# mgp25/OpenLTE

Hardware: AMD Instinct MI355X
Metric: DL subframes/sec @20MHz 100RB 64QAM, full chain FFT->CE->demap->rate-unmatch->turbo(REF)->CRC (SURVEY 8d W4) (higher is better)
Workload: dtype i8 IQ in, f32 FFT/CE/equaliser, i8 soft bits, i16 path metrics (differences exact modulo 2^16); 1 GPU; W4 full DL chain: 20 MHz/100 RB/64QAM, 9 allocations per subframe (8x12 PRB TBS 3240 + 1x4 PRB TBS 1064), 65536 subframes per GPU, int8 IQ in HBM; subframes_per_gpu=65536, N_ant=1, CFI=2, channel_estimate_form=compact, decoder=REF (reference-faithful, bit-exact), unique_subframes=96, streams_per_gpu=1

## Files before the change

### openlte_amd/csrc/turbo.hip

```cpp
#include <algorithm>
#include <cstring>
#include <initializer_list>
#include <type_traits>
#include <vector>

#include "plan_core.hpp"

using namespace turbo_geom;

namespace {

constexpr uint32_t RX_NULL_AS_INT = 10000;


__device__ __forceinline__ int sbyte(uint32_t w, int k) { return (int)__builtin_amdgcn_sbfe(w, 8 * k, 8); }

typedef __attribute__((address_space(3))) const uint8_t  lds_u8_t;
typedef __attribute__((address_space(3))) const int8_t   lds_i8_t;
typedef __attribute__((address_space(3))) const uint16_t lds_u16_t;
__device__ __forceinline__ uint32_t lds_u8(uint32_t addr) { return *(lds_u8_t *)(uintptr_t)addr; }
__device__ __forceinline__ int      lds_i8(uint32_t addr) { return *(lds_i8_t *)(uintptr_t)addr; }
__device__ __forceinline__ uint32_t lds_u16(uint32_t addr) { return *(lds_u16_t *)(uintptr_t)addr; }

typedef short v2s __attribute__((ext_vector_type(2)));
__device__ __forceinline__ v2s      as_v2s(uint32_t w) { return __builtin_bit_cast(v2s, w); }
__device__ __forceinline__ uint32_t as_u32(v2s v) { return __builtin_bit_cast(uint32_t, v); }
__device__ __forceinline__ v2s      even2(uint32_t w) { return (as_v2s(w) << 8) >> 8; }
__device__ __forceinline__ v2s      odd2(uint32_t w) { return as_v2s(w) >> 8; }
__device__ __forceinline__ uint32_t merge_bytes(v2s e, v2s o) { return __builtin_amdgcn_perm(as_u32(o), as_u32(e), 0x06020400u); }
__device__ __forceinline__ v2s      abs2(v2s a) { return __builtin_elementwise_max(a, (v2s)(0) - a); }
__device__ __forceinline__ uint32_t neg_mask(v2s d)
{
    uint32_t m;
    asm("v_pk_ashrrev_i16 %0, 15, %1 op_sel_hi:[0,1]" : "=v"(m) : "v"(as_u32(d)));
    return m;
}
__device__ __forceinline__ v2s bit_select(uint32_t m, v2s yes, v2s no) { return as_v2s((as_u32(yes) & m) | (as_u32(no) & ~m)); }
__device__ __forceinline__ v2s half_sum(v2s a, v2s b)
{
    uint32_t t = as_u32(a + b);
    asm("" : "+v"(t));
    return as_v2s(t) >> 1;
}

__device__ __forceinline__ int soft_xor(int a, int b)
{
    int mag = (abs(a) + abs(b)) >> 1;
    return ((a < 0) != (b < 0)) ? -mag : mag;
}


template <typename Op> __device__ __forceinline__ int wave_reduce_i(int v, Op op)
{
    v = op(v, __builtin_amdgcn_update_dpp(v, v, 0xB1, 0xF, 0xF, false));
    v = op(v, __builtin_amdgcn_update_dpp(v, v, 0x4E, 0xF, 0xF, false));
    v = op(v, __builtin_amdgcn_update_dpp(v, v, 0x141, 0xF, 0xF, false));
    v = op(v, __builtin_amdgcn_update_dpp(v, v, 0x140, 0xF, 0xF, false));
    return op(op(__builtin_amdgcn_readlane(v, 0), __builtin_amdgcn_readlane(v, 16)), op(__builtin_amdgcn_readlane(v, 32), __builtin_amdgcn_readlane(v, 48)));
}
__device__ __forceinline__ int      wave_max_i(int v) { return wave_reduce_i(v, [](int a, int b) { return max(a, b); }); }
__device__ __forceinline__ uint32_t wave_xor_u(uint32_t v) { return (uint32_t)wave_reduce_i((int)v, [](int a, int b) { return a ^ b; }); }
__device__ __forceinline__ float    wave_max_f(float v)
{
    return __int_as_float(wave_max_i(__float_as_int(v)));
}

__device__ __forceinline__ float block_max_abs_f(float v, float *red )
{
    v = wave_max_f(v);
    __syncthreads();
    if ((threadIdx.x & 63) == 0) red[threadIdx.x >> 6] = v;
    __syncthreads();
    float r = red[0];
    for (uint32_t w = 1; w < (blockDim.x >> 6); w++) r = fmaxf(r, red[w]);
    return r;
}
__device__ __forceinline__ int block_max_i(int v, int *red)
{
    v = wave_max_i(v);
    __syncthreads();
    if ((threadIdx.x & 63) == 0) red[threadIdx.x >> 6] = v;
    __syncthreads();
    int r = red[0];
    for (uint32_t w = 1; w < (blockDim.x >> 6); w++) r = max(r, red[w]);
    return r;
}

__device__ __forceinline__ void block_max_i2(int &a, int &b, int *red)
{
    a = wave_max_i(a); b = wave_max_i(b);
    __syncthreads();
    if ((threadIdx.x & 63) == 0) { red[threadIdx.x >> 6] = a; red[8 + (threadIdx.x >> 6)] = b; }
    __syncthreads();
    a = red[0]; b = red[8];
    for (uint32_t w = 1; w < (blockDim.x >> 6); w++) { a = max(a, red[w]); b = max(b, red[8 + w]); }
}

struct PrepOut { uint8_t *arr[6]; };

__device__ __forceinline__ uint4 pack16(const int (&q)[16])
{
    uint32_t w[4];
#pragma unroll
    for (int k = 0; k < 4; k++)
        w[k] = (uint32_t)(q[4 * k] & 0xFF) | ((uint32_t)(q[4 * k + 1] & 0xFF) << 8) | ((uint32_t)(q[4 * k + 2] & 0xFF) << 16) |
               ((uint32_t)(q[4 * k + 3] & 0xFF) << 24);
    return make_uint4(w[0], w[1], w[2], w[3]);
}
__device__ __forceinline__ size_t unit_off(size_t tile_off, uint32_t lane, uint32_t u)
{
    return tile_off + (size_t)(u >> 2) * 4096 + lane * 64 + (u & 3) * 16;
}
typedef uint32_t u32x4_t __attribute__((ext_vector_type(4)));
typedef __attribute__((address_space(4))) const u32x4_t const_u32x4_t;
__device__ __forceinline__ void load_idx16_at(const_u32x4_t *p , int nvalid, uint32_t (&idx)[16], uint32_t pad)
{
    const uint32_t pp = pad | (pad << 16);
    const u32x4_t  lo = p[0], hi = (nvalid > 8) ? p[1] : (u32x4_t)(pp);
    const uint32_t w[8] = {lo.x, lo.y, lo.z, lo.w, hi.x, hi.y, hi.z, hi.w};
#pragma unroll
    for (int k = 0; k < 16; k++) idx[k] = (w[k >> 1] >> (16 * (k & 1))) & 0xFFFFu;
}
__device__ __forceinline__ void load_idx16(const uint16_t *tab, uint32_t u, int nvalid, uint32_t (&idx)[16], uint32_t pad = 0)
{
    const uint4 *p = reinterpret_cast<const uint4 *>(tab + 16 * (size_t)u);
    const uint32_t pp = pad | (pad << 16);
    const uint4  lo = p[0], hi = (nvalid > 8) ? p[1] : make_uint4(pp, pp, pp, pp);
// ... 556 lines not shown
    auto closed = [](int W) { return W == 254 || W == 127; };
    auto closed16 = [](const uint32_t (&w)[16], int W) {
        uint32_t o[4];
#pragma unroll
        for (int j = 0; j < 4; j++) {
            const uint32_t p = pack4u(w[4 * j], w[4 * j + 1], w[4 * j + 2], w[4 * j + 3]);
            o[j] = W == 254 ? (p >> 1) & 0x7F7F7F7Fu : p;
        }
        return make_uint4(o[0], o[1], o[2], o[3]);
    };
    if (!(closed(w1max) && closed(w2max))) {
        const float W1 = (float)w1max, W2 = (float)w2max;
        for (uint32_t t = threadIdx.x; t < MTAB_N; t += blockDim.x) {
            const float w = (float)t;
            mtab1[t] = (int8_t)(int)(127.0f * (w / W1));
            mtab2[t] = (int8_t)(int)(127.0f * (w / W2));
        }
        __syncthreads();
    }
    if (nv >= 0) {
        *reinterpret_cast<uint4 *>(out.arr[4] + unit_off(tile_off, lane, u)) = closed(w1max) ? closed16(w1, w1max) : lookup16(0, w1);
        *reinterpret_cast<uint4 *>(out.arr[5] + unit_off(tile_off, lane, u)) = closed(w2max) ? closed16(w2, w2max) : lookup16(MTAB_N, w2);
    }
}


struct SisoPass {
    const uint8_t *in_a;
    const uint8_t *in_b;
    const uint8_t *mag;
    uint8_t       *out;
    uint32_t      *dec;
};
struct SisoArgs { SisoPass p[2]; };

typedef unsigned short v2u __attribute__((ext_vector_type(2)));
__device__ __forceinline__ uint32_t sign_bits(v2s n) { return __builtin_bit_cast(uint32_t, __builtin_bit_cast(v2u, n) >> 15); }

template <int S> __device__ __forceinline__ void acs_step2(v2s (&pm)[8], v2s x2, v2s y2, uint32_t &acc)
{
    const v2s mx = as_v2s(neg_mask(x2 ^ y2)), nmx = ~mx;
    const v2s uP = (x2 + y2) & nmx;
    const v2s uQ = (x2 - y2) & mx;
    const uint32_t m0p = neg_mask(x2) & 0xFFF8FFF8u;
    const v2s P2 = as_v2s(__builtin_amdgcn_bitop3_b32(as_u32(mx), m0p, 0xFFFCFFFCu, 0x06));
    const v2s Q2 = as_v2s(__builtin_amdgcn_bitop3_b32(as_u32(mx), m0p, 0xFFFCFFFCu, 0x60));
    const v2s n0 = pm[1] - pm[0], n1 = pm[3] - pm[2], n2 = pm[5] - pm[4], n3 = pm[7] - pm[6];
    constexpr uint32_t top = 0x00010001u << (15 - 4 * S);
    acc = __builtin_amdgcn_bitop3_b32(acc, neg_mask(n0), top, 0xF8);
    acc = __builtin_amdgcn_bitop3_b32(acc, neg_mask(n1), top >> 1, 0xF8);
    acc = __builtin_amdgcn_bitop3_b32(acc, neg_mask(n2), top >> 2, 0xF8);
    acc = __builtin_amdgcn_bitop3_b32(acc, neg_mask(n3), top >> 3, 0xF8);
    auto sel = [](v2s d, v2s yes, v2s no) { return bit_select(neg_mask(d), yes, no); };
    v2s nw[8];
    nw[0] = sel(n0 - P2, pm[1] + uP, pm[0] - uP);
    nw[4] = sel(n0 + P2, pm[1] - uP, pm[0] + uP);
    nw[1] = sel(n1 - Q2, pm[3] + uQ, pm[2] - uQ);
    nw[5] = sel(n1 + Q2, pm[3] - uQ, pm[2] + uQ);
    nw[2] = sel(n2 + Q2, pm[5] - uQ, pm[4] + uQ);
    nw[6] = sel(n2 - Q2, pm[5] + uQ, pm[4] - uQ);
    nw[3] = sel(n3 + P2, pm[7] - uP, pm[6] + uP);
    nw[7] = sel(n3 - P2, pm[7] + uP, pm[6] - uP);
#pragma unroll
    for (int s = 0; s < 8; s++) pm[s] = nw[s];
}

template <int R> __device__ __forceinline__ v2s byte_pair2(uint32_t w0, uint32_t w1)
{
    return as_v2s(__builtin_amdgcn_perm(w1, w0, (uint32_t)(4 + R) << 24 | 0x0C0000u | (uint32_t)R << 8 | 0x0Cu)) >> 7;
}

__device__ __forceinline__ uint32_t traceback_entry(uint32_t byte, uint32_t cur)
{
    uint32_t mask = 0;
    for (int k = 0; k < 2; k++) {
        const uint32_t nib = k ? byte >> 4 : byte & 15u;
        const uint32_t j = cur & 3u, bit = (nib >> (3 - j)) & 1u, st = 2 * j + bit;
        const bool     pos = (cur < st) || (cur == st && cur == 0);
        if (!pos) mask |= k ? 0x00FFu : 0xFF00u;
        cur = st;
    }
    return cur | mask << 8;
}
__device__ __forceinline__ uint32_t negate_bytes(uint32_t w, uint32_t m)
{
    const uint32_t x = w ^ m, y = m & 0x01010101u;
    return ((x & 0x7F7F7F7Fu) + y) ^ (x & 0x80808080u);
}

#ifndef SISO_WPE
#define SISO_WPE 4
#endif
template <bool MULTI>
__global__ __launch_bounds__(256) __attribute__((amdgpu_waves_per_eu(SISO_WPE, 8))) void k_turbo_siso(SisoArgs args, uint32_t K_arg, uint32_t n_tiles_arg, uint32_t mode, MultiArgs ma,
                                                                                                         const uint32_t *__restrict__ order)
{
    __shared__ uint32_t tb_lut[2048];
    for (uint32_t i = threadIdx.x; i < 2048; i += blockDim.x) tb_lut[i] = traceback_entry(i >> 3, i & 7u);
    __syncthreads();
    const uint32_t lane = threadIdx.x & 63u;
    uint32_t       K = K_arg, n_tiles = n_tiles_arg, wv = blockIdx.x * 4 + (threadIdx.x >> 6), n_wv = mode ? n_tiles : (n_tiles + 1) / 2;
    size_t         seg_off = 0;
    if constexpr (MULTI) {
        if (order) wv = __builtin_amdgcn_readfirstlane(order[wv]);
        if (wv >= n_tiles_arg) return;
        const_seg_t &sg = multi_seg(ma, wv);
        K = sg.K; n_tiles = sg.n_tiles; seg_off = sg.arr_off;
        wv -= mode ? sg.wv23 : sg.wv1;
        n_wv = mode ? n_tiles : (n_tiles + 1) / 2;
    }
    const uint32_t Kp = kpad64(K), nblk = Kp >> 6;
    if (wv >= n_wv) return;
    const uint8_t *pa[2], *pb[2], *pmag[2];
    uint8_t       *pout[2];
    uint32_t      *dec[2];
#pragma unroll
    for (int h = 0; h < 2; h++) {
        const SisoPass &ps   = args.p[mode ? h : 0];
        const uint32_t  tile = mode ? wv : min(2 * wv + h, n_tiles - 1);
        const size_t    off  = seg_off + (size_t)tile * Kp * 64 + lane * 64;
        pa[h] = ps.in_a + off; pb[h] = ps.in_b + off; pmag[h] = ps.mag + off; pout[h] = ps.out + off;
        dec[h] = ps.dec + (seg_off >> 3) + ((size_t)tile * nblk * 64 + lane) * 8;
    }

    v2s pm[8];
#pragma unroll
    for (int s = 0; s < 8; s++) pm[s] = (v2s)(0);

    uint4 A[2][4], B[2][4];
#pragma unroll
    for (int h = 0; h < 2; h++)
#pragma unroll
        for (int q = 0; q < 4; q++) {
            A[h][q] = reinterpret_cast<const uint4 *>(pa[h])[q];
            B[h][q] = reinterpret_cast<const uint4 *>(pb[h])[q];
        }
    for (uint32_t blk = 0; blk < nblk; blk++) {
        const uint32_t nxt = (blk + 1 < nblk) ? blk + 1 : blk;
        uint32_t       dw[2][8];
#pragma unroll
        for (int q = 0; q < 4; q++) {
#pragma unroll
            for (int g2 = 0; g2 < 2; g2++) {
                const int g = 2 * q + g2;
                uint32_t  acc_lo = 0, acc_hi = 0;
                if (blk * 64 + g * 8 < K) {
                    const uint32_t a0l = g2 ? A[0][q].z : A[0][q].x, a0h = g2 ? A[0][q].w : A[0][q].y;
                    const uint32_t a1l = g2 ? A[1][q].z : A[1][q].x, a1h = g2 ? A[1][q].w : A[1][q].y;
                    const uint32_t b0l = g2 ? B[0][q].z : B[0][q].x, b0h = g2 ? B[0][q].w : B[0][q].y;
                    const uint32_t b1l = g2 ? B[1][q].z : B[1][q].x, b1h = g2 ? B[1][q].w : B[1][q].y;
                    acs_step2<0>(pm, byte_pair2<0>(a0l, a1l), byte_pair2<0>(b0l, b1l), acc_lo);
                    acs_step2<1>(pm, byte_pair2<1>(a0l, a1l), byte_pair2<1>(b0l, b1l), acc_lo);
                    acs_step2<2>(pm, byte_pair2<2>(a0l, a1l), byte_pair2<2>(b0l, b1l), acc_lo);
                    acs_step2<3>(pm, byte_pair2<3>(a0l, a1l), byte_pair2<3>(b0l, b1l), acc_lo);
                    acs_step2<0>(pm, byte_pair2<0>(a0h, a1h), byte_pair2<0>(b0h, b1h), acc_hi);
                    acs_step2<1>(pm, byte_pair2<1>(a0h, a1h), byte_pair2<1>(b0h, b1h), acc_hi);
                    acs_step2<2>(pm, byte_pair2<2>(a0h, a1h), byte_pair2<2>(b0h, b1h), acc_hi);
                    acs_step2<3>(pm, byte_pair2<3>(a0h, a1h), byte_pair2<3>(b0h, b1h), acc_hi);
                }
                dw[0][g] = __builtin_amdgcn_perm(acc_lo, acc_hi, 0x05040100u);
                dw[1][g] = __builtin_amdgcn_perm(acc_lo, acc_hi, 0x07060302u);
            }
            if (q >= 2) {
#pragma unroll
                for (int qq = (q == 2 ? 0 : 3); qq <= (q == 2 ? 2 : 3); qq++)
#pragma unroll
                    for (int h = 0; h < 2; h++) {
                        A[h][qq] = reinterpret_cast<const uint4 *>(pa[h] + (size_t)nxt * 4096)[qq];
                        B[h][qq] = reinterpret_cast<const uint4 *>(pb[h] + (size_t)nxt * 4096)[qq];
                    }
            }
        }
#pragma unroll
        for (int h = 0; h < 2; h++) {
            uint4 *dp = reinterpret_cast<uint4 *>(dec[h] + (size_t)blk * 64 * 8);
            dp[0] = make_uint4(dw[h][0], dw[h][1], dw[h][2], dw[h][3]);
            dp[1] = make_uint4(dw[h][4], dw[h][5], dw[h][6], dw[h][7]);
        }
    }

    int cur[2] = {0, 0};
    {
        int best[2] = {0, 0};
#pragma unroll
        for (int s = 1; s < 8; s++) {
            const uint32_t d  = as_u32(pm[s] - pm[0]);
            const int      dh[2] = {(int)__builtin_amdgcn_sbfe(d, 0, 16), (int)d >> 16};
#pragma unroll
            for (int h = 0; h < 2; h++)
                if (dh[h] < best[h]) { best[h] = dh[h]; cur[h] = s; }
        }
    }

    uint4 M[2][4], Mn[2][4], D[2][2], Dn[2][2];
#pragma unroll
    for (int h = 0; h < 2; h++) {
        const uint4 *dp = reinterpret_cast<const uint4 *>(dec[h] + (size_t)(nblk - 1) * 64 * 8);
        D[h][0] = dp[0];
        D[h][1] = dp[1];
#pragma unroll
        for (int q = 0; q < 4; q++) M[h][q] = reinterpret_cast<const uint4 *>(pmag[h] + (size_t)(nblk - 1) * 4096)[q];
    }
    for (int blk = (int)nblk - 1; blk >= 0; blk--) {
        const int prv = blk > 0 ? blk - 1 : 0;
#pragma unroll
        for (int h = 0; h < 2; h++) {
            const uint4 *dpn = reinterpret_cast<const uint4 *>(dec[h] + (size_t)prv * 64 * 8);
            Dn[h][0] = dpn[0];
            Dn[h][1] = dpn[1];
#pragma unroll
            for (int q = 0; q < 4; q++) Mn[h][q] = reinterpret_cast<const uint4 *>(pmag[h] + (size_t)prv * 4096)[q];
        }
#pragma unroll
        for (int q = 3; q >= 0; q--) {
            uint32_t ow[2][4];
#pragma unroll
            for (int g2 = 1; g2 >= 0; g2--) {
                const int g = 2 * q + g2;
                uint32_t  o_hi[2] = {0, 0}, o_lo[2] = {0, 0};
                if ((uint32_t)blk * 64 + g * 8 < K) {
                    uint32_t word[2], mlo[2], mhi[2], msk[2][4];
#pragma unroll
                    for (int h = 0; h < 2; h++) {
                        const uint4 dq = D[h][g >> 2];
                        word[h] = (g & 3) == 0 ? dq.x : (g & 3) == 1 ? dq.y : (g & 3) == 2 ? dq.z : dq.w;
                        mlo[h]  = g2 ? M[h][q].z : M[h][q].x;
                        mhi[h]  = g2 ? M[h][q].w : M[h][q].y;
                    }
#pragma unroll
                    for (int b = 0; b < 4; b++) {
#pragma unroll
                        for (int h = 0; h < 2; h++) {
                            const uint32_t e = tb_lut[((word[h] >> (8 * b)) & 0xFFu) << 3 | (uint32_t)cur[h]];
                            cur[h]    = (int)(e & 7u);
                            msk[h][b] = e >> 8;
                        }
                    }
#pragma unroll
                    for (int h = 0; h < 2; h++) {
                        o_hi[h] = negate_bytes(mhi[h], msk[h][0] << 16 | msk[h][1]);
                        o_lo[h] = negate_bytes(mlo[h], msk[h][2] << 16 | msk[h][3]);
                    }
                }
#pragma unroll
                for (int h = 0; h < 2; h++) { ow[h][2 * g2] = o_lo[h]; ow[h][2 * g2 + 1] = o_hi[h]; }
            }
#pragma unroll
            for (int h = 0; h < 2; h++)
                reinterpret_cast<uint4 *>(pout[h] + (size_t)blk * 4096)[q] = make_uint4(ow[h][0], ow[h][1], ow[h][2], ow[h][3]);
        }
#pragma unroll
        for (int h = 0; h < 2; h++) {
            D[h][0] = Dn[h][0];
            D[h][1] = Dn[h][1];
#pragma unroll
            for (int q = 0; q < 4; q++) M[h][q] = Mn[h][q];
        }
    }
}

struct SmallPar { uint32_t cw, uw; };

__device__ __forceinline__ uint2 map_compose(uint2 F, uint2 G)
{
    return make_uint2(__builtin_amdgcn_perm(F.y, F.x, G.x), __builtin_amdgcn_perm(F.y, F.x, G.y));
}
__device__ __forceinline__ uint32_t map_at(uint2 F, uint32_t s) { return ((s & 4u ? F.y : F.x) >> (8 * (s & 3u))) & 7u; }
template <int N> __device__ __forceinline__ uint2 map_row_shl(uint2 v, uint2 keep)
{
    return make_uint2((uint32_t)__builtin_amdgcn_update_dpp((int)keep.x, (int)v.x, 0x100 + N, 0xF, 0xF, false),
                      (uint32_t)__builtin_amdgcn_update_dpp((int)keep.y, (int)v.y, 0x100 + N, 0xF, 0xF, false));
}

template <bool MULTI>
__global__ __launch_bounds__(64) void k_turbo_siso_small(SisoArgs args, uint32_t K_arg, uint32_t n_cb_arg, uint32_t mode, uint32_t gpw, MultiArgs ma)
{
    extern __shared__ __attribute__((aligned(16))) uint32_t sm_small[];
    SmallPar (*par)[64][4] = reinterpret_cast<SmallPar(*)[64][4]>(sm_small);
    uint32_t K = K_arg, n_cb = n_cb_arg, bidx = blockIdx.x;
    size_t   seg_off = 0;
    if constexpr (MULTI) {
        const_seg_t &sg = multi_seg(ma, blockIdx.x);
        K = sg.K; n_cb = sg.n_cb; seg_off = sg.arr_off; bidx = blockIdx.x - (mode ? sg.ws23 : sg.ws1);
    }
    const uint32_t Kp = kpad64(K), n_w32 = Kp >> 5;
    uint32_t      *decw = sm_small + gpw * 64 * 4 * 2;
    const uint32_t lane = threadIdx.x, gi = lane >> 2, j = lane & 3u;
    const uint32_t T0 = bidx * gpw, n_tr = n_cb * (mode ? 2u : 1u);
    const uint32_t n_g = min(gpw, n_tr - T0);
    auto pass_of = [&](uint32_t g) -> const SisoPass & { return args.p[mode ? (T0 + g) & 1u : 0u]; };
    auto off_of  = [&](uint32_t g) -> size_t {
        const uint32_t cb = mode ? (T0 + g) >> 1 : T0 + g;
        return seg_off + (size_t)(cb >> 6) * Kp * 64 + (cb & 63u) * 64;
    };
    const uint32_t n_chunk = (K + 63) >> 6;

    uint32_t XY = 0;
    uint32_t accv = 0;
    const uint32_t half_sel = j < 2 ? 0x01000100u : 0x03020302u;
#ifdef SMALL_PAD
    uint32_t padv[4] = {lane, lane + 1, lane + 2, lane + 3};
#endif
    int xs[SMALL_G], ys[SMALL_G];
    auto fetch = [&](uint32_t ch) {
#pragma unroll
        for (uint32_t g = 0; g < SMALL_G; g++)
            if (g < n_g) {
                const size_t e = off_of(g) + (size_t)ch * 4096 + lane;
                xs[g] = (int8_t)pass_of(g).in_a[e];
                ys[g] = (int8_t)pass_of(g).in_b[e];
            }
    };
    fetch(0);
    for (uint32_t ch = 0; ch < n_chunk; ch++) {
#pragma unroll
        for (uint32_t g = 0; g < SMALL_G; g++) {
            if (g >= n_g) break;
            const int      x  = xs[g], y = ys[g];
            const int      m0 = x >> 31, mx = m0 ^ (y >> 31), nmx = ~mx;
            const int      uP = ((x + y) << 1) & nmx, uQ = ((x - y) << 1) & mx;
            const int      c4 = (m0 & 8) - 4, P2 = c4 & nmx, Q2 = c4 & mx;
            auto pm16 = [](int v) { return ((uint32_t)v & 0xFFFFu) | ((uint32_t)(-v) << 16); };
            const uint32_t cP = pm16(P2), uPw = pm16(uP), cQ = pm16(Q2), uQw = pm16(uQ);
            auto swp = [](uint32_t w) { return (w >> 16) | (w << 16); };
// ... 6 lines not shown
        const uint32_t n_t = min(64u, K - ch * 64);
        if (gi < n_g) {
            auto steps8 = [&](uint32_t t8) {
                SmallPar pr[8];
#pragma unroll
                for (int k = 0; k < 8; k++) pr[k] = par[gi][t8 + k][j];
#pragma unroll
                for (int k = 0; k < 8; k++) {
                    const uint32_t t0 = (uint32_t)__builtin_amdgcn_mov_dpp((int)XY, 0x88, 0xF, 0xF, false);
                    const uint32_t t1 = (uint32_t)__builtin_amdgcn_mov_dpp((int)XY, 0xDD, 0xF, 0xF, false);
                    const v2s a = as_v2s(__builtin_amdgcn_perm(t0, t0, half_sel)), b = as_v2s(__builtin_amdgcn_perm(t1, t1, half_sel));
                    const v2s n = b - a;
                    accv = __builtin_amdgcn_alignbit(accv, as_u32(n), 31);
                    const v2s uw = as_v2s(pr[k].uw);
                    XY = as_u32(bit_select(neg_mask(n - as_v2s(pr[k].cw)), b + uw, a - uw));
#ifdef SMALL_PAD
#pragma unroll
                    for (int z = 0; z < SMALL_PAD; z++) asm volatile("v_add_u32 %0, %0, %1" : "+v"(padv[z & 3]) : "v"(lane));
#endif
                }
            };
            uint32_t t = 0;
            for (; t + 32 <= n_t; t += 32) {
                steps8(t); steps8(t + 8); steps8(t + 16); steps8(t + 24);
                decw[(gi * n_w32 + ((ch * 64 + t) >> 5)) * 4 + j] = accv;
            }
            if (t < n_t) {
                const uint32_t w = (ch * 64 + t) >> 5, left = n_t - t;
                for (; t < n_t; t += 8) steps8(t);
                decw[(gi * n_w32 + w) * 4 + j] = accv << (32u - left);
            }
        }
        __syncthreads();
    }

#ifdef SMALL_PAD
    if ((padv[0] ^ padv[1] ^ padv[2] ^ padv[3]) == 0x12345678u) decw[0] = 0;
#endif
    uint32_t cur = 0;
    {
        const uint32_t q0 = (uint32_t)__builtin_amdgcn_mov_dpp((int)XY, 0x00, 0xF, 0xF, false), q1 = (uint32_t)__builtin_amdgcn_mov_dpp((int)XY, 0x55, 0xF, 0xF, false);
        const uint32_t q2 = (uint32_t)__builtin_amdgcn_mov_dpp((int)XY, 0xAA, 0xF, 0xF, false), q3 = (uint32_t)__builtin_amdgcn_mov_dpp((int)XY, 0xFF, 0xF, 0xF, false);
        const short pm[8] = {(short)q0, (short)q1, (short)q2, (short)q3, (short)(q0 >> 16), (short)(q1 >> 16), (short)(q2 >> 16), (short)(q3 >> 16)};
        int best = 0;
#pragma unroll
        for (int st = 1; st < 8; st++) {
            const int d = (short)(pm[st] - pm[0]);
            if (d < best) { best = d; cur = st; }
        }
    }

    const uint2 MAP_ID = make_uint2(0x03020100u, 0x07060504u);
    for (uint32_t g = 0; g < n_g; g++) {
        uint32_t       end = (uint32_t)__builtin_amdgcn_readlane((int)cur, (int)(g * 4));
        const uint8_t *mag = pass_of(g).mag + off_of(g);
        uint8_t       *out = pass_of(g).out + off_of(g);
        uint8_t m_nxt = mag[(size_t)(n_chunk - 1) * 4096 + lane];
        for (int ch = (int)n_chunk - 1; ch >= 0; ch--) {
            const uint32_t t = (uint32_t)ch * 64 + lane;
            const uint8_t  m = m_nxt;
            if (ch > 0) m_nxt = mag[(size_t)(ch - 1) * 4096 + lane];
            const uint4    w = *reinterpret_cast<const uint4 *>(&decw[(g * n_w32 + (t >> 5)) * 4]);
            const uint32_t sh = 31u - (t & 31u);
            uint2          G = MAP_ID;
            if (t < K) {
                const uint32_t f = 0x06040200u + (((w.x >> sh) & 1u) | ((w.y >> sh) & 1u) << 8 | ((w.z >> sh) & 1u) << 16 | ((w.w >> sh) & 1u) << 24);
                G = make_uint2(f, f);
            }
            G = map_compose(G, map_row_shl<1>(G, MAP_ID));
            G = map_compose(G, map_row_shl<2>(G, MAP_ID));
            G = map_compose(G, map_row_shl<4>(G, MAP_ID));
            G = map_compose(G, map_row_shl<8>(G, MAP_ID));
            const uint32_t row = lane >> 4;
#pragma unroll
            for (int r = 1; r < 4; r++) {
                const uint2 R = make_uint2((uint32_t)__builtin_amdgcn_readlane((int)G.x, 16 * r), (uint32_t)__builtin_amdgcn_readlane((int)G.y, 16 * r));
                if (row < (uint32_t)r) G = map_compose(G, R);
            }
            const uint2    Gn  = make_uint2((uint32_t)__shfl_down((int)G.x, 1u), (uint32_t)__shfl_down((int)G.y, 1u));
            const uint32_t nxt = lane == 63 ? end : map_at(Gn, end);
            const uint32_t st  = map_at(G, end);
            if (t < K) {
                const bool    pos = (nxt < st) || (nxt == st && nxt == 0);
                out[(size_t)ch * 4096 + lane] = pos ? m : (uint8_t)(0u - m);
            }
            end = (uint32_t)__builtin_amdgcn_readlane((int)st, 0);
        }
    }
}

struct SM { v2s m; uint32_t s; };
__device__ __forceinline__ SM   to_sm(v2s x) { return SM{abs2(x), neg_mask(x)}; }
__device__ __forceinline__ v2s  to_tc(const SM &a) { return as_v2s(as_u32(a.m) ^ a.s) - as_v2s(a.s); }
__device__ __forceinline__ SM   sxor_sm(const SM &a, const SM &b) { return SM{half_sum(a.m, b.m), a.s ^ b.s}; }
struct UnitWords { uint32_t w[5]; };
__device__ __forceinline__ UnitWords load_unit_words(const uint8_t *arr, size_t tile_off, uint32_t lane, uint32_t u)
{
    const uint4 c    = *reinterpret_cast<const uint4 *>(arr + unit_off(tile_off, lane, u));
    uint32_t    prev = 0x7F7F7F7Fu;
    if (u > 0) prev = *reinterpret_cast<const uint32_t *>(arr + unit_off(tile_off, lane, u - 1) + 12);
    return UnitWords{{prev, c.x, c.y, c.z, c.w}};
}
struct WordPairs { v2s et, ot; SM e, o; };
__device__ __forceinline__ WordPairs word_pairs(uint32_t w)
{
    const v2s e = even2(w), o = odd2(w);
    return WordPairs{e, o, to_sm(e), to_sm(o)};
}
__device__ __forceinline__ SM delay_sm(const SM &cur, const SM &prev)
{
    return SM{as_v2s(__builtin_amdgcn_alignbit(as_u32(cur.m), as_u32(prev.m), 16)), __builtin_amdgcn_alignbit(cur.s, prev.s, 16)};
}
struct SX { v2s tc, m; uint32_t s; };
__device__ __forceinline__ SX sxor_full(const SM &a, const SM &b)
{
    const SM  r  = sxor_sm(a, b);
    const v2s tc = to_tc(r);
    return SX{tc, r.m, neg_mask(tc)};
}
__device__ __forceinline__ void feedback_sm(const WordPairs &cur, const WordPairs &prev, SX &fe, SX &fo)
{
    const SM d2e = delay_sm(cur.e, prev.e), d2o = delay_sm(cur.o, prev.o);
    fe = sxor_full(d2e, prev.o);
    fo = sxor_full(d2o, d2e);
}
__device__ __forceinline__ v2s sxor_tc(const SM &a, const SX &f) { return to_tc(SM{half_sum(a.m, f.m), a.s ^ f.s}); }

struct PermArgs { const uint8_t *A1; const uint8_t *X2; uint8_t *out[2];  };

#ifndef PERM_NB
#define PERM_NB 4
#endif
static_assert(PERM_NB == PERM_BLOCKS, "a size's perm grid is a multiple of 128 workgroups (the merged decode's map granularity) only for four blocks per workgroup");
template <int NSLOT, bool MULTI = false>
__global__ __launch_bounds__(384) void k_turbo_perm(PermArgs a, uint32_t K_arg, uint32_t n_cb_arg, const uint16_t *__restrict__ pi_arg, MultiArgs ma)
{
    static_assert(NSLOT == 1, "one unit per thread");
    uint32_t K = K_arg, n_cb = n_cb_arg, bidx = blockIdx.x, grid = gridDim.x;
    size_t   seg_off = 0;
    const uint16_t *__restrict__ pi = pi_arg;
    if constexpr (MULTI) {
        const_seg_t &sg = multi_seg(ma, blockIdx.x >> 7);
        K = sg.K; n_cb = sg.n_cb; pi = (const uint16_t *)sg.pi; bidx = blockIdx.x - sg.wg_perm; grid = sg.perm_grid;
        seg_off = sg.arr_off;
    }
    extern __shared__ __attribute__((aligned(16))) int8_t smp[];
    int8_t *mtab = smp, *sm = smp + MTAB_N;
    const uint32_t Kp = kpad64(K), n_units = Kp >> 4;
    int           *red_i = reinterpret_cast<int *>(sm + Kp);
    const uint32_t u0 = threadIdx.x;
    const int      nv = (u0 < n_units) ? min(16, max(0, (int)K - 16 * (int)u0)) : -1;
    IdxRaw         praw;
    {
        const uint4 *ip = reinterpret_cast<const uint4 *>(pi + 16 * (size_t)(nv > 0 ? u0 : 0));
        const uint32_t kk = K | K << 16;
        praw.lo = ip[0];
        praw.hi = (nv > 8) ? ip[1] : make_uint4(kk, kk, kk, kk);
    }
#pragma unroll 1
    for (uint32_t it = 0; it < PERM_NB; it++) {
        const uint32_t cb = xcd_cb(bidx + it * grid, n_cb), tile = cb >> 6, lane = cb & 63;
        const size_t   tile_off = seg_off + (size_t)tile * Kp * 64;
        if (cb >= n_cb) {
            if (MULTI && cb < ((n_cb + 63u) & ~63u) && nv >= 0) {
                *reinterpret_cast<uint4 *>(a.out[0] + unit_off(tile_off, lane, u0)) = make_uint4(0, 0, 0, 0);
                *reinterpret_cast<uint4 *>(a.out[1] + unit_off(tile_off, lane, u0)) = make_uint4(0, 0, 0, 0);
            }
            continue;
        }
        uint32_t u = u0;
        asm volatile("" : "+v"(u), "+v"(praw.lo.x), "+v"(praw.lo.y), "+v"(praw.lo.z), "+v"(praw.lo.w), "+v"(praw.hi.x), "+v"(praw.hi.y), "+v"(praw.hi.z), "+v"(praw.hi.w));
        uint4          X2 = make_uint4(0, 0, 0, 0);
        if (nv >= 0) {
            const UnitWords wa = load_unit_words(a.A1, tile_off, lane, u);
            WordPairs       pa = word_pairs(wa.w[0]);
            X2 = *reinterpret_cast<const uint4 *>(a.X2 + unit_off(tile_off, lane, u));
            uint32_t c1[4];
#pragma unroll
            for (int j = 0; j < 4; j++) {
                const WordPairs ca = word_pairs(wa.w[j + 1]);
                SX              fe, fo;
                feedback_sm(ca, pa, fe, fo);
                c1[j] = (4 * j < nv) ? merge_bytes(sxor_tc(ca.e, fe), sxor_tc(ca.o, fo)) : 0u;
                pa    = ca;
            }
            *reinterpret_cast<uint4 *>(sm + 16 * u) = make_uint4(c1[0], c1[1], c1[2], c1[3]);
        }
        __syncthreads();
        uint4 I1 = make_uint4(0, 0, 0, 0);
        if (nv > 0) {
            uint32_t idx[16];
            unpack_idx16(praw, idx);
            I1 = gather16_bytes(MTAB_N, idx);
        }
        if (nv >= 0) *reinterpret_cast<uint4 *>(a.out[0] + unit_off(tile_off, lane, u)) = I1;
        uint32_t w[16], wm = 0;
        if (nv <= 0) X2 = make_uint4(0, 0, 0, 0);
        abs_sum16(X2, I1, w, wm);
        const int   wmax = block_max_i((int)wm, red_i);
        if (wmax == 254 || wmax == 127) {
            uint32_t o[4];
#pragma unroll
            for (int j = 0; j < 4; j++) {
                const uint32_t p = pack4u(w[4 * j], w[4 * j + 1], w[4 * j + 2], w[4 * j + 3]);
                o[j] = wmax == 254 ? (p >> 1) & 0x7F7F7F7Fu : p;
            }
            if (nv >= 0) *reinterpret_cast<uint4 *>(a.out[1] + unit_off(tile_off, lane, u)) = make_uint4(o[0], o[1], o[2], o[3]);
            continue;
        }
        const float W = (float)wmax;
        for (uint32_t t = threadIdx.x; t < MTAB_N; t += blockDim.x) mtab[t] = (int8_t)(int)(127.0f * ((float)t / W));
        __syncthreads();
        if (nv >= 0) *reinterpret_cast<uint4 *>(a.out[1] + unit_off(tile_off, lane, u)) = lookup16(0, w);
        __syncthreads();
    }
}

struct VoteArgs { const uint8_t *X0, *A1, *B1, *B2; };

template <bool GROUP, int NSLOT, bool MULTI = false>
__global__ __launch_bounds__(384) __attribute__((amdgpu_waves_per_eu(6, 8))) void k_turbo_vote(VoteArgs a, uint32_t K_arg, uint32_t n_cb_arg, const uint16_t *__restrict__ inv_arg,
                                                    uint8_t *__restrict__ c_bits, GroupDesc g, MultiArgs ma)
{
    static_assert(NSLOT == 1, "one unit per thread");
    uint32_t K = K_arg, n_cb = n_cb_arg, bidx = blockIdx.x;
    size_t   seg_off = 0;
    const uint16_t *__restrict__ inv = inv_arg;
    if constexpr (MULTI) {
        const_seg_t &sg = multi_seg(ma, blockIdx.x >> 9);
        K = sg.K; n_cb = sg.n_cb; inv = (const uint16_t *)sg.inv2; bidx = blockIdx.x - sg.wg_cb; seg_off = sg.arr_off;
        g.desc += sg.cb_base;
    }
    extern __shared__ __attribute__((aligned(16))) int8_t sm[];
    const uint32_t cb = xcd_cb(bidx, n_cb), tile = cb >> 6, lane = cb & 63, Kp = kpad64(K), n_units = Kp >> 4;
    if (cb >= n_cb) return;
    const size_t   tile_off = seg_off + (size_t)tile * Kp * 64;
    int8_t        *d12 = sm, *bits = sm + 2 * Kp + 32;
    uint32_t      *red_u = reinterpret_cast<uint32_t *>(bits + Kp);
    const uint32_t u  = threadIdx.x;
    const int      nv = (u < n_units) ? min(16, max(0, (int)K - 16 * (int)u)) : -1;
    IdxRaw vraw;
    {
        const uint4 *ip = reinterpret_cast<const uint4 *>(inv + 16 * (size_t)(nv > 0 ? u : 0));
        vraw.lo = ip[0];
        vraw.hi = ip[1];
    }
    const uint32_t crc_w0 = (GROUP && nv > 0) ? g.crc_tab[MI_CRC_TAB_BIAS + K - 16 * u - 16] : 0u;
    v2s            s0e[4], s0o[4];
    if (threadIdx.x == 0) *reinterpret_cast<uint32_t *>(d12 + 2 * Kp) = 0u;
    if (nv >= 0) {
        const UnitWords wa = load_unit_words(a.A1, tile_off, lane, u), wb = load_unit_words(a.B1, tile_off, lane, u),
                        wc = load_unit_words(a.B2, tile_off, lane, u);
        WordPairs       pa = word_pairs(wa.w[0]), pb = word_pairs(wb.w[0]), pc = word_pairs(wc.w[0]);
        const uint4    x0 = *reinterpret_cast<const uint4 *>(a.X0 + unit_off(tile_off, lane, u));
        const uint32_t x0w[4] = {x0.x, x0.y, x0.z, x0.w};
        uint32_t       dn[8];
#pragma unroll
        for (int j = 0; j < 4; j++) {
            const WordPairs ca = word_pairs(wa.w[j + 1]), cb1 = word_pairs(wb.w[j + 1]), cb2 = word_pairs(wc.w[j + 1]);
            SX              fe, fo, ge, go, he, ho;
            feedback_sm(ca, pa, fe, fo);
            feedback_sm(cb1, pb, ge, go);
            feedback_sm(cb2, pc, he, ho);
            v2s d[2];
#pragma unroll
            for (int h = 0; h < 2; h++) {
                const SM  &A = h ? ca.o : ca.e, &B = h ? cb1.o : cb1.e, &B_ = h ? cb2.o : cb2.e;
                const SX  &G = h ? go : ge, &G_ = h ? ho : he;
                const v2s  At = h ? ca.ot : ca.et;
                const v2s dAG = At - G.tc, t = as_v2s(as_u32(dAG) ^ B.s) - as_v2s(B.s);
                const v2s v1  = bit_select(B.s ^ G.s, (v2s)(0) - (t >> 1), half_sum(B.m, G.m));
                const v2s v2  = bit_select(B_.s ^ G_.s, (v2s)(0) - ((B_.m - G_.tc) >> 1), half_sum(B_.m, G_.m));
                d[h] = v1 + v2;
                const v2s c1 = sxor_tc(A, h ? fo : fe);
                (h ? s0o[j] : s0e[j]) = (h ? odd2(x0w[j]) : even2(x0w[j])) + c1;
            }
            pa = ca; pb = cb1; pc = cb2;
            const bool in = 4 * j < nv;
            dn[2 * j]     = in ? __builtin_amdgcn_perm(as_u32(d[1]), as_u32(d[0]), 0x05040100u) : 0u;
            dn[2 * j + 1] = in ? __builtin_amdgcn_perm(as_u32(d[1]), as_u32(d[0]), 0x07060302u) : 0u;
        }
        uint4 *dst = reinterpret_cast<uint4 *>(d12 + 32 * u);
        dst[0] = make_uint4(dn[0], dn[1], dn[2], dn[3]);
        dst[1] = make_uint4(dn[4], dn[5], dn[6], dn[7]);
    } else {
#pragma unroll
        for (int j = 0; j < 4; j++) s0e[j] = s0o[j] = (v2s)(0);
    }
    __syncthreads();
    uint32_t alloc = 0, tbs = 0, F = 0, crc = 0;
    if (GROUP) {
        alloc = g.desc[cb].alloc;
        tbs   = g.desc[cb].tbs;
        F     = K - tbs - 24;
    }
    if (nv > 0) {
        const uint32_t  iw[8] = {vraw.lo.x, vraw.lo.y, vraw.lo.z, vraw.lo.w, vraw.hi.x, vraw.hi.y, vraw.hi.z, vraw.hi.w};
        uint32_t        me[4], mo[4], bw[4];
#pragma unroll
        for (int j = 0; j < 4; j++) {
            const uint32_t i0 = iw[2 * j] & 0xFFFFu, i1 = iw[2 * j] >> 16, i2 = iw[2 * j + 1] & 0xFFFFu, i3 = iw[2 * j + 1] >> 16;
            const uint32_t ge = lds_u16(i0) | lds_u16(i2) << 16, go = lds_u16(i1) | lds_u16(i3) << 16;
            me[j] = as_u32((s0e[j] + as_v2s(ge)) >> 15);
            mo[j] = as_u32((s0o[j] + as_v2s(go)) >> 15);
            bw[j] = (me[j] & 0x00010001u) | (mo[j] & 0x00010001u) << 8;
        }
        if (GROUP) {
            if (!(nv == 16 && 16 * u >= F)) {
#pragma unroll
                for (int j = 0; j < 4; j++) {
                    auto ok = [&](int k) { return (k < nv && 16 * u + k >= F) ? 0xFFFFu : 0u; };
                    me[j] &= ok(4 * j) | ok(4 * j + 2) << 16;
                    mo[j] &= ok(4 * j + 1) | ok(4 * j + 3) << 16;
                }
            }
            const uint32_t GS = 0x864CFBu << 8;
            uint32_t       w = crc_w0;
#pragma unroll
            for (int k = 15; k >= 0; k--) {
                const int      j = k >> 2;
                const uint32_t m = (k & 3) == 0 ? (uint32_t)__builtin_amdgcn_sbfe(me[j], 0, 1) : (k & 3) == 1 ? (uint32_t)__builtin_amdgcn_sbfe(mo[j], 0, 1)
                                 : (k & 3) == 2 ? (uint32_t)((int)me[j] >> 31) : (uint32_t)((int)mo[j] >> 31);
                crc ^= w & m;
                if (k > 0) w = (w << 1) ^ ((uint32_t)((int)w >> 31) & GS);
            }
        }
        const uint4 pk = make_uint4(bw[0], bw[1], bw[2], bw[3]);
        if (GROUP) *reinterpret_cast<uint4 *>(bits + 16 * u) = pk;
        else {
            uint2 *o = reinterpret_cast<uint2 *>(c_bits + (size_t)cb * K + 16 * u);
            o[0] = make_uint2(pk.x, pk.y);
            if (nv > 8) o[1] = make_uint2(pk.z, pk.w);
        }
    }
    if (GROUP) {
        crc = wave_xor_u(crc);
        __syncthreads();
        if ((threadIdx.x & 63) == 0) red_u[threadIdx.x >> 6] = crc;
        __syncthreads();
        crc = 0;
        for (uint32_t w = 0; w < (blockDim.x >> 6); w++) crc ^= red_u[w];
        if (threadIdx.x == 0) g.status[alloc] = (crc == 0) ? 0  : 2 ;
        uint8_t *o = g.out_bits + (size_t)alloc * g.out_stride;
        if (g.packed && ((F | tbs) & 7u) == 0) {
            const uint32_t nby = tbs >> 3, nw = nby >> 2;
            auto byte_at = [&](uint32_t m) -> uint32_t {
                const uint2 w = *reinterpret_cast<const uint2 *>(bits + F + 8 * m);
                return (((w.x * 0x08040201u) >> 24) & 0xFu) << 4 | (((w.y * 0x08040201u) >> 24) & 0xFu);
            };
            for (uint32_t m = threadIdx.x; m < nw; m += blockDim.x)
                reinterpret_cast<uint32_t *>(o)[m] = byte_at(4 * m) | byte_at(4 * m + 1) << 8 | byte_at(4 * m + 2) << 16 | byte_at(4 * m + 3) << 24;
            for (uint32_t m = 4 * nw + threadIdx.x; m < nby; m += blockDim.x) o[m] = (uint8_t)byte_at(m);
        } else if (g.packed) {
            for (uint32_t m = threadIdx.x; m < (tbs + 7) >> 3; m += blockDim.x) {
                uint32_t v = 0;
                for (uint32_t b = 0; b < 8; b++) v = v << 1 | ((8 * m + b < tbs) ? ((uint32_t)bits[F + 8 * m + b] & 1u) : 0u);
                o[m] = (uint8_t)v;
            }
        } else if ((F & 3u) == 0) {
            const uint32_t nq = tbs >> 2;
            const uint32_t *bw = reinterpret_cast<const uint32_t *>(bits + F);
            for (uint32_t m = threadIdx.x; m < nq; m += blockDim.x) reinterpret_cast<uint32_t *>(o)[m] = bw[m];
            for (uint32_t m = 4 * nq + threadIdx.x; m < tbs; m += blockDim.x) o[m] = (uint8_t)bits[m + F];
// ... 594 lines not shown
```

Measured before the change: 2.722 million subframes/s.

## Switch turbo soft bits to sign-magnitude SWAR byte arithmetic

Soft bits exchanged between the turbo SISO traceback and the permutation/extrinsic kernels become sign-magnitude bytes instead of two's complement. All four bytes of a word are then processed at once with SWAR helpers in a new header, replacing the earlier split into even/odd packed 16-bit lanes. Feedback delays, soft-XOR and the step-10/11 combinations are rewritten as biased byte-wise operations. The goal is fewer VALU instructions per word, at the cost of an encoding change that every producer and consumer must agree on to stay bit-exact.

```diff
diff --git a/openlte_amd/csrc/turbo.hip b/openlte_amd/csrc/turbo.hip
--- a/openlte_amd/csrc/turbo.hip
+++ b/openlte_amd/csrc/turbo.hip
@@ -5,6 +5,7 @@
 #include <vector>
 
 #include "plan_core.hpp"
+#include "turbo_swar.h"
 
 using namespace turbo_geom;
 
@@ -25,10 +26,6 @@
 typedef short v2s __attribute__((ext_vector_type(2)));
 __device__ __forceinline__ v2s      as_v2s(uint32_t w) { return __builtin_bit_cast(v2s, w); }
 __device__ __forceinline__ uint32_t as_u32(v2s v) { return __builtin_bit_cast(uint32_t, v); }
-__device__ __forceinline__ v2s      even2(uint32_t w) { return (as_v2s(w) << 8) >> 8; }
-__device__ __forceinline__ v2s      odd2(uint32_t w) { return as_v2s(w) >> 8; }
-__device__ __forceinline__ uint32_t merge_bytes(v2s e, v2s o) { return __builtin_amdgcn_perm(as_u32(o), as_u32(e), 0x06020400u); }
-__device__ __forceinline__ v2s      abs2(v2s a) { return __builtin_elementwise_max(a, (v2s)(0) - a); }
 __device__ __forceinline__ uint32_t neg_mask(v2s d)
 {
     uint32_t m;
@@ -36,13 +33,6 @@
     return m;
 }
 __device__ __forceinline__ v2s bit_select(uint32_t m, v2s yes, v2s no) { return as_v2s((as_u32(yes) & m) | (as_u32(no) & ~m)); }
-__device__ __forceinline__ v2s half_sum(v2s a, v2s b)
-{
-    uint32_t t = as_u32(a + b);
-    asm("" : "+v"(t));
-    return as_v2s(t) >> 1;
-}
-
 __device__ __forceinline__ int soft_xor(int a, int b)
 {
     int mag = (abs(a) + abs(b)) >> 1;
@@ -765,11 +755,6 @@
     }
     return cur | mask << 8;
 }
-__device__ __forceinline__ uint32_t negate_bytes(uint32_t w, uint32_t m)
-{
-    const uint32_t x = w ^ m, y = m & 0x01010101u;
-    return ((x & 0x7F7F7F7Fu) + y) ^ (x & 0x80808080u);
-}
 
 #ifndef SISO_WPE
 #define SISO_WPE 4
@@ -921,8 +906,8 @@
                     }
 #pragma unroll
                     for (int h = 0; h < 2; h++) {
-                        o_hi[h] = negate_bytes(mhi[h], msk[h][0] << 16 | msk[h][1]);
-                        o_lo[h] = negate_bytes(mlo[h], msk[h][2] << 16 | msk[h][3]);
+                        o_hi[h] = turbo_swar::joined_from(mhi[h], msk[h][0] << 16 | msk[h][1]);
+                        o_lo[h] = turbo_swar::joined_from(mlo[h], msk[h][2] << 16 | msk[h][3]);
                     }
                 }
 #pragma unroll
@@ -1095,17 +1080,14 @@
             const uint32_t st  = map_at(G, end);
             if (t < K) {
                 const bool    pos = (nxt < st) || (nxt == st && nxt == 0);
-                out[(size_t)ch * 4096 + lane] = pos ? m : (uint8_t)(0u - m);
+                out[(size_t)ch * 4096 + lane] = (pos || m == 0) ? m : (uint8_t)(m | 0x80u);
             }
             end = (uint32_t)__builtin_amdgcn_readlane((int)st, 0);
         }
     }
 }
 
-struct SM { v2s m; uint32_t s; };
-__device__ __forceinline__ SM   to_sm(v2s x) { return SM{abs2(x), neg_mask(x)}; }
-__device__ __forceinline__ v2s  to_tc(const SM &a) { return as_v2s(as_u32(a.m) ^ a.s) - as_v2s(a.s); }
-__device__ __forceinline__ SM   sxor_sm(const SM &a, const SM &b) { return SM{half_sum(a.m, b.m), a.s ^ b.s}; }
+namespace sw = turbo_swar;
 struct UnitWords { uint32_t w[5]; };
 __device__ __forceinline__ UnitWords load_unit_words(const uint8_t *arr, size_t tile_off, uint32_t lane, uint32_t u)
 {
@@ -1114,31 +1096,6 @@
     if (u > 0) prev = *reinterpret_cast<const uint32_t *>(arr + unit_off(tile_off, lane, u - 1) + 12);
     return UnitWords{{prev, c.x, c.y, c.z, c.w}};
 }
-struct WordPairs { v2s et, ot; SM e, o; };
-__device__ __forceinline__ WordPairs word_pairs(uint32_t w)
-{
-    const v2s e = even2(w), o = odd2(w);
-    return WordPairs{e, o, to_sm(e), to_sm(o)};
-}
-__device__ __forceinline__ SM delay_sm(const SM &cur, const SM &prev)
-{
-    return SM{as_v2s(__builtin_amdgcn_alignbit(as_u32(cur.m), as_u32(prev.m), 16)), __builtin_amdgcn_alignbit(cur.s, prev.s, 16)};
-}
-struct SX { v2s tc, m; uint32_t s; };
-__device__ __forceinline__ SX sxor_full(const SM &a, const SM &b)
-{
-    const SM  r  = sxor_sm(a, b);
-    const v2s tc = to_tc(r);
-    return SX{tc, r.m, neg_mask(tc)};
-}
-__device__ __forceinline__ void feedback_sm(const WordPairs &cur, const WordPairs &prev, SX &fe, SX &fo)
-{
-    const SM d2e = delay_sm(cur.e, prev.e), d2o = delay_sm(cur.o, prev.o);
-    fe = sxor_full(d2e, prev.o);
-    fo = sxor_full(d2o, d2e);
-}
-__device__ __forceinline__ v2s sxor_tc(const SM &a, const SX &f) { return to_tc(SM{half_sum(a.m, f.m), a.s ^ f.s}); }
-
 struct PermArgs { const uint8_t *A1; const uint8_t *X2; uint8_t *out[2];  };
 
 #ifndef PERM_NB
@@ -1186,16 +1143,15 @@
         uint4          X2 = make_uint4(0, 0, 0, 0);
         if (nv >= 0) {
             const UnitWords wa = load_unit_words(a.A1, tile_off, lane, u);
-            WordPairs       pa = word_pairs(wa.w[0]);
+            uint32_t        pa = wa.w[0];
             X2 = *reinterpret_cast<const uint4 *>(a.X2 + unit_off(tile_off, lane, u));
             uint32_t c1[4];
 #pragma unroll
             for (int j = 0; j < 4; j++) {
-                const WordPairs ca = word_pairs(wa.w[j + 1]);
-                SX              fe, fo;
-                feedback_sm(ca, pa, fe, fo);
-                c1[j] = (4 * j < nv) ? merge_bytes(sxor_tc(ca.e, fe), sxor_tc(ca.o, fo)) : 0u;
-                pa    = ca;
+                const uint32_t ja = wa.w[j + 1];
+                const sw::SM4  A  = sw::unjoin(ja);
+                c1[j] = (4 * j < nv) ? sw::to_tc(sw::step3(A, sw::feedback(ja, pa))) : 0u;
+                pa    = ja;
             }
             *reinterpret_cast<uint4 *>(sm + 16 * u) = make_uint4(c1[0], c1[1], c1[2], c1[3]);
         }
@@ -1264,34 +1220,26 @@
     if (nv >= 0) {
         const UnitWords wa = load_unit_words(a.A1, tile_off, lane, u), wb = load_unit_words(a.B1, tile_off, lane, u),
                         wc = load_unit_words(a.B2, tile_off, lane, u);
-        WordPairs       pa = word_pairs(wa.w[0]), pb = word_pairs(wb.w[0]), pc = word_pairs(wc.w[0]);
+        uint32_t        pa = wa.w[0], pb = wb.w[0], pc = wc.w[0];
         const uint4    x0 = *reinterpret_cast<const uint4 *>(a.X0 + unit_off(tile_off, lane, u));
         const uint32_t x0w[4] = {x0.x, x0.y, x0.z, x0.w};
         uint32_t       dn[8];
 #pragma unroll
         for (int j = 0; j < 4; j++) {
-            const WordPairs ca = word_pairs(wa.w[j + 1]), cb1 = word_pairs(wb.w[j + 1]), cb2 = word_pairs(wc.w[j + 1]);
-            SX              fe, fo, ge, go, he, ho;
-            feedback_sm(ca, pa, fe, fo);
-            feedback_sm(cb1, pb, ge, go);
-            feedback_sm(cb2, pc, he, ho);
-            v2s d[2];
-#pragma unroll
-            for (int h = 0; h < 2; h++) {
-                const SM  &A = h ? ca.o : ca.e, &B = h ? cb1.o : cb1.e, &B_ = h ? cb2.o : cb2.e;
-                const SX  &G = h ? go : ge, &G_ = h ? ho : he;
-                const v2s  At = h ? ca.ot : ca.et;
-                const v2s dAG = At - G.tc, t = as_v2s(as_u32(dAG) ^ B.s) - as_v2s(B.s);
-                const v2s v1  = bit_select(B.s ^ G.s, (v2s)(0) - (t >> 1), half_sum(B.m, G.m));
-                const v2s v2  = bit_select(B_.s ^ G_.s, (v2s)(0) - ((B_.m - G_.tc) >> 1), half_sum(B_.m, G_.m));
-                d[h] = v1 + v2;
-                const v2s c1 = sxor_tc(A, h ? fo : fe);
-                (h ? s0o[j] : s0e[j]) = (h ? odd2(x0w[j]) : even2(x0w[j])) + c1;
-            }
-            pa = ca; pb = cb1; pc = cb2;
+            const uint32_t ja = wa.w[j + 1], jb = wb.w[j + 1], jc = wc.w[j + 1];
+            const sw::SM4  A = sw::unjoin(ja), B = sw::unjoin(jb), B_ = sw::unjoin(jc);
+            const sw::SM4  F  = sw::feedback(ja, pa);
+            const sw::SM4  G  = sw::feedback(jb, pb);
+            const sw::SM4  G_ = sw::feedback(jc, pc);
+            pa = ja; pb = jb; pc = jc;
+            const uint32_t u1 = sw::step10_biased(A, B, G), n2 = sw::step11_neg_biased(B_, G_);
+            const uint32_t de = sw::sub_halves(sw::even_halves(u1), sw::even_halves(n2)), dd = sw::sub_halves(sw::odd_halves(u1), sw::odd_halves(n2));
+            const uint32_t x0b = x0w[j] ^ sw::HI, nc = sw::step3_neg_biased(A, F);
+            s0e[j] = as_v2s(sw::sub_halves(sw::even_halves(x0b), sw::even_halves(nc)));
+            s0o[j] = as_v2s(sw::sub_halves(sw::odd_halves(x0b), sw::odd_halves(nc)));
             const bool in = 4 * j < nv;
-            dn[2 * j]     = in ? __builtin_amdgcn_perm(as_u32(d[1]), as_u32(d[0]), 0x05040100u) : 0u;
-            dn[2 * j + 1] = in ? __builtin_amdgcn_perm(as_u32(d[1]), as_u32(d[0]), 0x07060302u) : 0u;
+            dn[2 * j]     = in ? __builtin_amdgcn_perm(dd, de, 0x05040100u) : 0u;
+            dn[2 * j + 1] = in ? __builtin_amdgcn_perm(dd, de, 0x07060302u) : 0u;
         }
         uint4 *dst = reinterpret_cast<uint4 *>(d12 + 32 * u);
         dst[0] = make_uint4(dn[0], dn[1], dn[2], dn[3]);
diff --git a/openlte_amd/csrc/turbo_swar.h b/openlte_amd/csrc/turbo_swar.h
--- /dev/null
+++ b/openlte_amd/csrc/turbo_swar.h
@@ -0,0 +1,96 @@
+#pragma once
+
+#include <cstdint>
+
+#ifdef __HIPCC__
+#define SWAR_FN __host__ __device__ __forceinline__
+#else
+#define SWAR_FN inline
+#endif
+
+namespace turbo_swar {
+
+constexpr uint32_t HI = 0x80808080u, LO7 = 0x7F7F7F7Fu, ONES = 0x01010101u, EVEN = 0x00FF00FFu;
+
+SWAR_FN uint32_t alignbit(uint32_t hi, uint32_t lo, uint32_t sh)
+{
+#if defined(__HIP_DEVICE_COMPILE__)
+    return __builtin_amdgcn_alignbit(hi, lo, sh);
+#else
+    return (uint32_t)((((uint64_t)hi << 32) | lo) >> sh);
+#endif
+}
+SWAR_FN uint32_t sub_halves(uint32_t a, uint32_t b)
+{
+#if defined(__HIP_DEVICE_COMPILE__)
+    typedef short v2s_t __attribute__((ext_vector_type(2)));
+    return __builtin_bit_cast(uint32_t, __builtin_bit_cast(v2s_t, a) - __builtin_bit_cast(v2s_t, b));
+#else
+    return ((a - (b & 0xFFFFu)) & 0xFFFFu) | ((a & 0xFFFF0000u) - (b & 0xFFFF0000u));
+#endif
+}
+
+struct SM4 { uint32_t m, s; };
+
+SWAR_FN uint32_t low7(uint32_t bits) { return bits - (bits >> 7); }
+
+SWAR_FN uint32_t to_joined(uint32_t w)
+{
+    const uint32_t s = w & HI, t = s >> 7;
+    return (w ^ (s - t)) + t;
+}
+SWAR_FN uint32_t joined_from(uint32_t m, uint32_t neg_mask) { return m | (neg_mask & (m + LO7) & HI); }
+SWAR_FN SM4 unjoin(uint32_t j) { return SM4{j & LO7, j & HI}; }
+SWAR_FN SM4 split(uint32_t w) { return unjoin(to_joined(w)); }
+SWAR_FN uint32_t join(const SM4 &a) { return a.m | a.s; }
+SWAR_FN uint32_t to_tc(const SM4 &a)
+{
+    const uint32_t t = a.s >> 7;
+    return ((a.m ^ (a.s - t)) + t) | a.s;
+}
+
+SWAR_FN uint32_t biased(uint32_t x, uint32_t neg)
+{
+    const uint32_t t = neg >> 7;
+    return ((x ^ (neg - t)) + t) + (neg ^ HI);
+}
+SWAR_FN uint32_t even_halves(uint32_t w) { return w & EVEN; }
+SWAR_FN uint32_t odd_halves(uint32_t w) { return (w >> 8) & EVEN; }
+
+SWAR_FN uint32_t half_sum(uint32_t ma, uint32_t mb) { return ((ma + mb) >> 1) & LO7; }
+SWAR_FN SM4 soft_xor(const SM4 &a, const SM4 &b)
+{
+    const uint32_t m = half_sum(a.m, b.m);
+    return SM4{m, (a.s ^ b.s) & (m + LO7) & HI};
+}
+
+SWAR_FN uint32_t delay2(uint32_t cur, uint32_t prev) { return alignbit(cur, prev, 16); }
+SWAR_FN uint32_t delay3(uint32_t cur, uint32_t prev) { return alignbit(cur, prev, 8); }
+SWAR_FN SM4 feedback(uint32_t cur_joined, uint32_t prev_joined)
+{
+    const uint32_t d2 = delay2(cur_joined, prev_joined), d3 = delay3(cur_joined, prev_joined);
+    const uint32_t x = d2 ^ d3;
+    const uint32_t m = (d2 & d3 & LO7) + ((x >> 1) & 0x3F3F3F3Fu);
+    return SM4{m, x & (m + LO7) & HI};
+}
+
+SWAR_FN SM4 step3(const SM4 &A, const SM4 &F) { return soft_xor(A, F); }
+SWAR_FN uint32_t step3_neg_biased(const SM4 &A, const SM4 &F) { return biased(half_sum(A.m, F.m), A.s ^ F.s ^ HI); }
+
+SWAR_FN uint32_t avg_biased(uint32_t xb, uint32_t yb) { return (xb & yb) + (((xb ^ yb) >> 1) & LO7); }
+
+SWAR_FN uint32_t step10_biased(const SM4 &A, const SM4 &B, const SM4 &G)
+{
+    const uint32_t mx = B.s ^ G.s, tm = mx >> 7, m7 = mx - tm;
+    const uint32_t y  = (A.m & m7) | (B.m & ~m7);
+    const uint32_t w  = avg_biased(G.m | HI, biased(y, mx & (A.s ^ B.s)));
+    return (w ^ (m7 | mx)) + tm;
+}
+SWAR_FN uint32_t step11_neg_biased(const SM4 &B, const SM4 &G)
+{
+    const uint32_t mx = B.s ^ G.s, tm = mx >> 7, m7 = mx - tm;
+    const uint32_t w  = avg_biased(B.m | HI, biased(G.m, mx & B.s));
+    return (w ^ ~(m7 | mx)) + (tm ^ ONES);
+}
+
+}
```

Result: faster. 2.798 million subframes/s (median of 6 runs) (+2.8%).
